# lim0606/pytorch-ardae-vae

Measured on AMD Instinct MI355X. Metric: AR-DAE-VAE train-steps/sec (batch 512, nz_cdae 256) on dbMNIST, higher is better.
Workload: dtype f32; 1 GPU; BASELINE config #2: MNISTIPVAE mlp z=32 h=256 + cDAE mlp-grad h=256 L=3, global batch 512, nz_cdae 256 (131072 rows), dynamic binarisation on device, 1 cDAE + 1 VAE update per step; global_batch=512, nz_cdae=256, per_gpu_batch=512, parallelism=dp1

## Files before the change

### pytorch-ardae-vae_amd/csrc/wgrad_x9.hip

```cpp
#include <stdlib.h>

#include <type_traits>

#include "profile.h"
#include "wgrad.h"
#include "wgrad_wide_tiles.h"

namespace ardae {
namespace {

typedef __bf16 bf16x8 __attribute__((ext_vector_type(8)));
typedef float f32x8 __attribute__((ext_vector_type(8)));

constexpr int XT = 256;
constexpr int XRC = 16;
constexpr int X_PLANE_BYTES = 2 * XT * 16;
constexpr int X_OP_BYTES = 3 * X_PLANE_BYTES;
constexpr int X_BUF_BYTES = 2 * X_OP_BYTES;

__device__ __forceinline__ void xload1(float& dst, unsigned voff, const float* sbase) {
  asm volatile("s_nop 4\n\tglobal_load_dword %0, %1, %2" : "+v"(dst) : "v"(voff), "s"(sbase) : "memory");
}
__device__ __forceinline__ void xload4(f32x4& dst, unsigned voff, const float* sbase) {
  asm volatile("s_nop 4\n\tglobal_load_dwordx4 %0, %1, %2" : "+v"(dst) : "v"(voff), "s"(sbase) : "memory");
}
template <int N>
__device__ __forceinline__ void xwait() { asm volatile("s_waitcnt vmcnt(%0)" : : "n"(N) : "memory"); }
__device__ __forceinline__ void take_landed(const float& loaded, unsigned& top, float& copy) {
  asm volatile("v_and_b32 %0, 0xffff0000, %2\n\tv_mov_b32 %1, %2" : "=&v"(top), "=&v"(copy) : "v"(loaded));
}
__device__ __forceinline__ void take_landed(const f32x4& loaded, f32x4& copy) {
  asm volatile("v_mov_b32 %0, %4\n\tv_mov_b32 %1, %5\n\tv_mov_b32 %2, %6\n\tv_mov_b32 %3, %7"
               : "=&v"(copy[0]), "=&v"(copy[1]), "=&v"(copy[2]), "=&v"(copy[3])
               : "v"(loaded[0]), "v"(loaded[1]), "v"(loaded[2]), "v"(loaded[3]));
}

struct Cut3 { unsigned h, m, l; };
__device__ __forceinline__ Cut3 cut3(float x) {
  Cut3 c;
  c.h = __float_as_uint(x) & 0xffff0000u;
  const float r1 = x - __uint_as_float(c.h);
  c.m = __float_as_uint(r1) & 0xffff0000u;
  c.l = __float_as_uint(r1 - __uint_as_float(c.m));
  return c;
}
__device__ __forceinline__ unsigned pack_hi(unsigned even, unsigned odd) { return __builtin_amdgcn_perm(odd, even, 0x07060302u); }
typedef unsigned u32x4 __attribute__((ext_vector_type(4)));

template <int N, class F>
__device__ __forceinline__ void static_for(F&& f) {
  if constexpr (N > 0) {
    static_for<N - 1>(f);
    f(std::integral_constant<int, N - 1>{});
  }
}
constexpr int X9_PA[9] = {2, 1, 2, 0, 2, 1, 0, 1, 0}, X9_PB[9] = {2, 2, 1, 2, 0, 1, 1, 0, 0};

struct X9Chunk {
  const float* g; const float* x; const float* rs;
  int ldg, ldx;
  float fb, fr;
};

__global__ __launch_bounds__(256, 1) void wgrad_x9_kernel(const WwBatchDev batch) {
  extern __shared__ __attribute__((aligned(16))) unsigned char lds[];
  const int tid = threadIdx.x, lane = tid & 63;
  const int wave = __builtin_amdgcn_readfirstlane(tid >> 6);
  const int l31 = lane & 31, hh = lane >> 5;
  const int wo = wave >> 1, wi = wave & 1;
  const int ti = (int)blockIdx.x / batch.splits, split = (int)blockIdx.x - ti * batch.splits;
  const WwTile T = batch.t[ti];

  const int cpp = T.M / XRC;
  const int ctot = cpp * T.npairs;
  const int cps = (ctot + batch.splits - 1) / batch.splits;
  const int c_begin = split * cps;
  const int c_end = c_begin + cps < ctot ? c_begin + cps : ctot;

  auto chunk_at = [&](int ch) {
    X9Chunk c;
    const int cc = ch < c_end ? ch : c_end - 1;
    const int pr = cc >= cpp ? 1 : 0;
    const int m0 = (cc - pr * cpp) * XRC;
    c.ldg = pr ? T.ldG[1] : T.ldG[0];
    c.ldx = pr ? T.ldX[1] : T.ldX[0];
    c.g = (pr ? T.G[1] : T.G[0]) + (size_t)m0 * c.ldg + T.o0;
    c.x = (pr ? T.X[1] : T.X[0]) + (size_t)m0 * c.ldx + T.i0;
    const bool vec = T.want_vec && pr == T.bias_pair && ch < c_end;
    c.fb = vec ? 1.f : 0.f;
    c.fr = (vec && T.rowscale) ? 1.f : 0.f;
    c.rs = T.rowscale ? T.rowscale + m0 : c.g;
    return c;
  };
  auto issue_loads = [&](const X9Chunk& c, float (&g)[XRC], float (&x)[XRC], f32x4 (&rs)[4]) {
    const float* pg = c.g;
    const float* px = c.x;
#pragma unroll
    for (int j = 0; j < XRC; ++j) {
      xload1(g[j], (unsigned)tid * 4u, pg); pg += c.ldg;
      if ((j & 3) == 3) xload4(rs[j >> 2], 0u, c.rs + (j & ~3));
    }
#pragma unroll
    for (int j = 0; j < XRC; ++j) { xload1(x[j], (unsigned)tid * 4u, px); px += c.ldx; }
  };
  float bsum = 0.f, rsum = 0.f;
  auto write_group = [&](const u32x4& h, const u32x4& m, const u32x4& l, int op, int kg, unsigned char* buf) {
    unsigned char* p = buf + op * X_OP_BYTES + (kg * XT + tid) * 16;
    *reinterpret_cast<u32x4*>(p) = h;
    *reinterpret_cast<u32x4*>(p + X_PLANE_BYTES) = m;
    *reinterpret_cast<u32x4*>(p + 2 * X_PLANE_BYTES) = l;
  };
  auto stage_group = [&](const float (&v)[XRC], int op, int kg, unsigned char* buf) {
    u32x4 h, m, l;
#pragma unroll
    for (int q = 0; q < 4; ++q) {
      const Cut3 e = cut3(v[8 * kg + 2 * q]), o = cut3(v[8 * kg + 2 * q + 1]);
      h[q] = pack_hi(e.h, o.h); m[q] = pack_hi(e.m, o.m); l[q] = pack_hi(e.l, o.l);
    }
    write_group(h, m, l, op, kg, buf);
  };

  f32x16 acc[4][4];
#pragma unroll
  for (int a = 0; a < 4; ++a)
#pragma unroll
    for (int b = 0; b < 4; ++b)
#pragma unroll
      for (int r = 0; r < 16; ++r) acc[a][b][r] = 0.f;

  if (c_begin < c_end) {
    float gc[XRC], xc[XRC];
    f32x4 rsc[4];
#pragma unroll
    for (int j = 0; j < XRC; ++j) gc[j] = xc[j] = 0.f;
#pragma unroll
    for (int q = 0; q < 4; ++q) rsc[q] = f32x4{0.f, 0.f, 0.f, 0.f};
    {
      const X9Chunk c0 = chunk_at(c_begin);
      issue_loads(c0, gc, xc, rsc);
      asm volatile("s_waitcnt vmcnt(0)" ::: "memory");
#pragma unroll
      for (int j = 0; j < XRC; ++j) asm volatile("" : "+v"(gc[j]), "+v"(xc[j]));
#pragma unroll
      for (int q = 0; q < 4; ++q) asm volatile("" : "+v"(rsc[q]));
      {
        float s0 = 0.f, r0 = 0.f;
#pragma unroll
        for (int j = 0; j < XRC; ++j) { s0 += gc[j]; r0 += gc[j] * rsc[j >> 2][j & 3]; }
        bsum += s0 * c0.fb; rsum += r0 * c0.fr;
      }
      stage_group(gc, 0, 0, lds); stage_group(gc, 0, 1, lds); stage_group(xc, 1, 0, lds); stage_group(xc, 1, 1, lds);
      issue_loads(chunk_at(c_begin + 1), gc, xc, rsc);
      __syncthreads();
    }
    int buf = 0;
    bf16x8 Af[3][4], Bf[3][4];
    auto read_plane = [&](auto pp, const unsigned char* from) {
      constexpr int p = decltype(pp)::value;
      static_for<4>([&](auto aa) {
        constexpr int a = decltype(aa)::value;
        Af[p][a] = *reinterpret_cast<const bf16x8*>(from + p * X_PLANE_BYTES + (hh * XT + wo * 128 + a * 32 + l31) * 16);
      });
      static_for<4>([&](auto bb) {
        constexpr int b = decltype(bb)::value;
        Bf[p][b] = *reinterpret_cast<const bf16x8*>(from + X_OP_BYTES + p * X_PLANE_BYTES + (hh * XT + wi * 128 + b * 32 + l31) * 16);
      });
    };
    using I0 = std::integral_constant<int, 0>;
    using I1 = std::integral_constant<int, 1>;
    using I2 = std::integral_constant<int, 2>;
    read_plane(I2{}, lds);
    read_plane(I1{}, lds);
    X9Chunk c1 = chunk_at(c_begin + 1);
#pragma unroll 1
    for (int ch = c_begin; ch < c_end; ++ch) {
      unsigned char* cur = lds + buf * X_BUF_BYTES;
      unsigned char* oth = lds + (buf ^ 1) * X_BUF_BYTES;
      const X9Chunk c2 = chunk_at(ch + 2);
      const float* pgn = c2.g;
      const float* pxn = c2.x;
      u32x4 sh, sm, sl;
      Cut3 ce{0u, 0u, 0u}, co{0u, 0u, 0u};
      float r1 = 0.f, vv = 0.f, cs = 0.f, cr = 0.f;
      f32x4 rsv = {0.f, 0.f, 0.f, 0.f};
      static_for<144>([&](auto nn) {
        constexpr int n = decltype(nn)::value, s = n >> 4, idx = n & 15, a = idx >> 2, b = idx & 3;
        acc[a][b] = __builtin_amdgcn_mfma_f32_32x32x16_bf16(Af[X9_PA[s]][a], Bf[X9_PB[s]][b], acc[a][b], 0, 0, 0);
        __builtin_amdgcn_sched_barrier(0);
        if constexpr (n == 0) {
          read_plane(I0{}, cur);
          __builtin_amdgcn_sched_barrier(0);
        }
        if constexpr (n < 124) {
          constexpr int grp = n / 31, r = n % 31;
          if constexpr (r < 28) {
            constexpr int pr = r / 7, slot = r % 7, e = 8 * grp + 2 * pr + (slot >= 3 ? 1 : 0), op = e >> 4, j = e & 15;
            float& v = op ? xc[j] : gc[j];
            if constexpr (slot == 0 || slot == 3) {
              xwait<35>();
              Cut3& c = slot == 0 ? ce : co;
              take_landed(v, c.h, vv);
              r1 = vv - __uint_as_float(c.h);
              if constexpr (op == 0) cs += vv;
            } else if constexpr (slot == 1 || slot == 4) {
              Cut3& c = slot == 1 ? ce : co;
              c.m = __float_as_uint(r1) & 0xffff0000u;
              c.l = __float_as_uint(r1 - __uint_as_float(c.m));
              if constexpr (op == 0) {
                if constexpr ((j & 3) == 0) { xwait<31>(); take_landed(rsc[j >> 2], rsv); }
                cr += vv * rsv[j & 3];
              }
            } else if constexpr (slot == 2 || slot == 5) {
              if constexpr (op == 0) {
                xload1(v, (unsigned)tid * 4u, pgn); pgn += c2.ldg;
                if constexpr ((j & 3) == 3) xload4(rsc[j >> 2], 0u, c2.rs + (j & ~3));
              } else {
                xload1(v, (unsigned)tid * 4u, pxn); pxn += c2.ldx;
              }
            } else {
              sh[pr] = pack_hi(ce.h, co.h); sm[pr] = pack_hi(ce.m, co.m); sl[pr] = pack_hi(ce.l, co.l);
            }
          } else {
            constexpr int pl = r - 28;
            unsigned char* p = oth + (grp >> 1) * X_OP_BYTES + ((grp & 1) * XT + tid) * 16 + pl * X_PLANE_BYTES;
            *reinterpret_cast<u32x4*>(p) = pl == 0 ? sh : pl == 1 ? sm : sl;
          }
          __builtin_amdgcn_sched_barrier(0);
        }
        if constexpr (n == 124) {
          __syncthreads();
          __builtin_amdgcn_sched_barrier(0);
        }
        if constexpr (n == 125) {
          read_plane(I2{}, oth);
          __builtin_amdgcn_sched_barrier(0);
        }
        if constexpr (n == 128) {
          read_plane(I1{}, oth);
          __builtin_amdgcn_sched_barrier(0);
        }
      });
      bsum += cs * c1.fb; rsum += cr * c1.fr;
      buf ^= 1;
      c1 = c2;
    }
    asm volatile("s_waitcnt vmcnt(0)" ::: "memory");
  }

  float* __restrict__ part = T.partial + (size_t)split * T.O * T.I;
#pragma unroll
  for (int a = 0; a < 4; ++a) {
#pragma unroll
    for (int b = 0; b < 4; ++b) {
      const int i = T.i0 + wi * 128 + b * 32 + l31;
#pragma unroll
      for (int r = 0; r < 16; ++r) {
        const int o = T.o0 + wo * 128 + a * 32 + (r & 3) + 8 * (r >> 2) + 4 * hh;
        part[(size_t)o * T.I + i] = acc[a][b][r];
      }
    }
  }
  if (T.want_vec && T.i0 == 0) {
    T.partial_vec[((size_t)split * 2 + 0) * T.O + T.o0 + tid] = bsum;
    T.partial_vec[((size_t)split * 2 + 1) * T.O + T.o0 + tid] = rsum;
  }
}

}

bool wgrad_x9_eligible(const WgradProblem& p) {
  static const bool off = debug_knob("ARDAE_WGRAD_X9") && atoi(debug_knob("ARDAE_WGRAD_X9")) == 0;
  if (off || p.O % XT || p.I % XT || p.M % XRC || p.M < 64 * 32) return false;
  for (int k = 0; k < p.npairs; ++k)
    if ((int64_t)p.ldG[k] * XRC * 4 >= (int64_t)1 << 31 || (int64_t)p.ldX[k] * XRC * 4 >= (int64_t)1 << 31) return false;
  return true;
}

int launch_wgrad_x9(const WwBatchDev& b, hipStream_t st) {
  static const bool attr_set = [] {
    return hipFuncSetAttribute(reinterpret_cast<const void*>(wgrad_x9_kernel), hipFuncAttributeMaxDynamicSharedMemorySize, 2 * X_BUF_BYTES) == hipSuccess;
  }();
  ARDAE_CHECK_ARG(attr_set, "wgrad_x9: cannot reserve %d bytes of LDS", 2 * X_BUF_BYTES);
  hipLaunchKernelGGL(wgrad_x9_kernel, dim3(b.ntiles * b.splits), dim3(256), 2 * X_BUF_BYTES, st, b);
  return 0;
}

}
```

### scratch/x9_stamps_patch.py

```python
import sys
p='pytorch-ardae-vae_amd/csrc/wgrad_wide_tiles.h'
s=open(p).read()
s=s.replace('  int ntiles, splits;','  int ntiles, splits;\n  unsigned long long* stamps;')
open(p,'w').write(s)
p='pytorch-ardae-vae_amd/csrc/wgrad_x9.hip'
s=open(p).read()
s=s.replace('''      unsigned char* cur = lds + buf * X_BUF_BYTES;''','''      const bool stamp = batch.stamps && blockIdx.x == 7 && ch == c_begin + 20 && tid == 0;
      unsigned long long T0 = 0, T1 = 0, T2 = 0, T3 = 0, TM[9] = {0};
      if (batch.stamps) T0 = __builtin_readcyclecounter();
      unsigned char* cur = lds + buf * X_BUF_BYTES;''',1)
s=s.replace('''        constexpr int n = decltype(nn)::value, s = n >> 4, idx = n & 15, a = idx >> 2, b = idx & 3;''','''        constexpr int n = decltype(nn)::value, s = n >> 4, idx = n & 15, a = idx >> 2, b = idx & 3;
        if constexpr (n == 1) { if (batch.stamps) T1 = __builtin_readcyclecounter(); }
        if constexpr (idx == 15) { if (batch.stamps) TM[s] = __builtin_readcyclecounter(); }
        if constexpr (n == 143) { if (batch.stamps) T2 = __builtin_readcyclecounter(); }''',1)
s=s.replace('''      bsum += cs * c1.fb; rsum += cr * c1.fr;
      buf ^= 1;''','''      bsum += cs * c1.fb; rsum += cr * c1.fr;
      buf ^= 1;
      if (batch.stamps) T3 = __builtin_readcyclecounter();
      if (stamp) { batch.stamps[0] = T0; batch.stamps[1] = T1; batch.stamps[2] = T2; batch.stamps[3] = T3; batch.stamps[4] = __builtin_readcyclecounter(); batch.stamps[5] = __builtin_amdgcn_s_memrealtime();
                   for (int q = 0; q < 9; ++q) batch.stamps[8 + q] = TM[q]; }
      if (batch.stamps && blockIdx.x == 7 && ch == c_begin + 120 && tid == 0) { batch.stamps[6] = __builtin_readcyclecounter(); batch.stamps[7] = __builtin_amdgcn_s_memrealtime(); }''',1)
s=s.replace('''int launch_wgrad_x9(const WwBatchDev& b, hipStream_t st) {''','''int launch_wgrad_x9(const WwBatchDev& b0, hipStream_t st) {
  static unsigned long long* dstamps = nullptr;
  static int calls = 0;
  WwBatchDev b = b0;
  b.stamps = nullptr;
  if (debug_knob("ARDAE_X9_STAMPS")) {
    if (!dstamps) { (void)hipMalloc(&dstamps, 256); (void)hipMemset(dstamps, 0, 256); }
    b.stamps = dstamps;
    if (++calls == 40) {
      (void)hipDeviceSynchronize();
      unsigned long long h[32];
      (void)hipMemcpy(h, dstamps, 256, hipMemcpyDeviceToHost);
      fprintf(stderr, "x9 stamps (cycles): start->MFMA1 %llu, MFMA1->MFMA143 %llu, ->end of trip %llu, barrier %llu; 100 trips: %llu cycles, %llu ticks of 100 MHz; products:", h[1] - h[0], h[2] - h[1], h[3] - h[2], h[4] - h[3], h[6] - h[4], h[7] - h[5]);
      for (int q = 0; q < 9; ++q) fprintf(stderr, " %llu", h[8 + q] - (q ? h[8 + q - 1] : h[1]));
      fprintf(stderr, "\\n");
    }
  }''',1)
open(p,'w').write(s)
```

Measured before the change: 223.5 train-steps/sec.

## Re-schedule x9 wgrad main loop: split LDS stores, spread fragment reads, hoist per-trip setup

New measurement: 225.5 train-steps/sec, median of 6. About the same (+0.9%).

```diff
diff --git a/pytorch-ardae-vae_amd/csrc/wgrad_x9.hip b/pytorch-ardae-vae_amd/csrc/wgrad_x9.hip
--- a/pytorch-ardae-vae_amd/csrc/wgrad_x9.hip
+++ b/pytorch-ardae-vae_amd/csrc/wgrad_x9.hip
@@ -46,6 +46,7 @@
 }
 __device__ __forceinline__ unsigned pack_hi(unsigned even, unsigned odd) { return __builtin_amdgcn_perm(odd, even, 0x07060302u); }
 typedef unsigned u32x4 __attribute__((ext_vector_type(4)));
+typedef unsigned u32x2 __attribute__((ext_vector_type(2)));
 
 template <int N, class F>
 __device__ __forceinline__ void static_for(F&& f) {
@@ -77,19 +78,26 @@
   const int c_begin = split * cps;
   const int c_end = c_begin + cps < ctot ? c_begin + cps : ctot;
 
+  const float fb_on = T.want_vec ? 1.f : 0.f, fr_on = (T.want_vec && T.rowscale) ? 1.f : 0.f;
+  auto chunk_rows = [&](int ch, int& pr, int& m0) {
+    const int cc = ch < c_end ? ch : c_end - 1;
+    pr = cc >= cpp ? 1 : 0;
+    m0 = (cc - pr * cpp) * XRC;
+  };
+  auto chunk_ld = [&](int ch, X9Chunk& c, int pr) {
+    c.ldg = pr ? T.ldG[1] : T.ldG[0];
+    c.ldx = pr ? T.ldX[1] : T.ldX[0];
+    const bool vec = (pr == T.bias_pair) & (ch < c_end);
+    c.fb = vec ? fb_on : 0.f;
+    c.fr = vec ? fr_on : 0.f;
+  };
+  auto chunk_g = [&](X9Chunk& c, int pr, int m0) { c.g = (pr ? T.G[1] : T.G[0]) + (size_t)m0 * c.ldg + T.o0; };
+  auto chunk_x = [&](X9Chunk& c, int pr, int m0) { c.x = (pr ? T.X[1] : T.X[0]) + (size_t)m0 * c.ldx + T.i0; };
+  auto chunk_rs = [&](X9Chunk& c, int m0) { c.rs = T.rowscale ? T.rowscale + m0 : c.g; };
   auto chunk_at = [&](int ch) {
     X9Chunk c;
-    const int cc = ch < c_end ? ch : c_end - 1;
-    const int pr = cc >= cpp ? 1 : 0;
-    const int m0 = (cc - pr * cpp) * XRC;
-    c.ldg = pr ? T.ldG[1] : T.ldG[0];
-    c.ldx = pr ? T.ldX[1] : T.ldX[0];
-    c.g = (pr ? T.G[1] : T.G[0]) + (size_t)m0 * c.ldg + T.o0;
-    c.x = (pr ? T.X[1] : T.X[0]) + (size_t)m0 * c.ldx + T.i0;
-    const bool vec = T.want_vec && pr == T.bias_pair && ch < c_end;
-    c.fb = vec ? 1.f : 0.f;
-    c.fr = (vec && T.rowscale) ? 1.f : 0.f;
-    c.rs = T.rowscale ? T.rowscale + m0 : c.g;
+    int pr, m0;
+    chunk_rows(ch, pr, m0); chunk_ld(ch, c, pr); chunk_g(c, pr, m0); chunk_x(c, pr, m0); chunk_rs(c, m0);
     return c;
   };
   auto issue_loads = [&](const X9Chunk& c, float (&g)[XRC], float (&x)[XRC], f32x4 (&rs)[4]) {
@@ -153,46 +161,48 @@
       issue_loads(chunk_at(c_begin + 1), gc, xc, rsc);
       __syncthreads();
     }
-    int buf = 0;
     bf16x8 Af[3][4], Bf[3][4];
-    auto read_plane = [&](auto pp, const unsigned char* from) {
-      constexpr int p = decltype(pp)::value;
-      static_for<4>([&](auto aa) {
-        constexpr int a = decltype(aa)::value;
-        Af[p][a] = *reinterpret_cast<const bf16x8*>(from + p * X_PLANE_BYTES + (hh * XT + wo * 128 + a * 32 + l31) * 16);
-      });
-      static_for<4>([&](auto bb) {
-        constexpr int b = decltype(bb)::value;
-        Bf[p][b] = *reinterpret_cast<const bf16x8*>(from + X_OP_BYTES + p * X_PLANE_BYTES + (hh * XT + wi * 128 + b * 32 + l31) * 16);
-      });
+    auto read_frag = [&](auto pp, auto kk, const unsigned char* from) {
+      constexpr int p = decltype(pp)::value, k = decltype(kk)::value;
+      if constexpr (k < 4) Af[p][k] = *reinterpret_cast<const bf16x8*>(from + p * X_PLANE_BYTES + (hh * XT + wo * 128 + k * 32 + l31) * 16);
+      else Bf[p][k - 4] = *reinterpret_cast<const bf16x8*>(from + X_OP_BYTES + p * X_PLANE_BYTES + (hh * XT + wi * 128 + (k - 4) * 32 + l31) * 16);
     };
     using I0 = std::integral_constant<int, 0>;
     using I1 = std::integral_constant<int, 1>;
     using I2 = std::integral_constant<int, 2>;
-    read_plane(I2{}, lds);
-    read_plane(I1{}, lds);
-    X9Chunk c1 = chunk_at(c_begin + 1);
+    static_for<8>([&](auto kk) { read_frag(I2{}, kk, lds); });
+    static_for<8>([&](auto kk) { read_frag(I1{}, kk, lds); });
+    X9Chunk c2 = chunk_at(c_begin + 2);
+    const float* pgn = c2.g;
+    const float* pxn = c2.x;
+    float fb1, fr1;
+    { const X9Chunk c1 = chunk_at(c_begin + 1); fb1 = c1.fb; fr1 = c1.fr; }
+    unsigned char* cur = lds;
+    unsigned char* oth = lds + X_BUF_BYTES;
+    u32x4 sh, sm, sl;
+    Cut3 ce{0u, 0u, 0u}, co{0u, 0u, 0u};
+    float r1 = 0.f, vv = 0.f, cs = 0.f, cr = 0.f;
+    f32x4 rsv = {0.f, 0.f, 0.f, 0.f};
+    int npr = 0, nm0 = 0;
+    auto store_half = [&](auto gg, auto pl_, auto half_) {
+      constexpr int grp = decltype(gg)::value, pl = decltype(pl_)::value, half = decltype(half_)::value;
+      unsigned char* p = oth + (grp >> 1) * X_OP_BYTES + ((grp & 1) * XT + tid) * 16 + pl * X_PLANE_BYTES + half * 8;
+      const u32x4& v = pl == 0 ? sh : pl == 1 ? sm : sl;
+      *reinterpret_cast<u32x2*>(p) = u32x2{v[2 * half], v[2 * half + 1]};
+    };
 #pragma unroll 1
     for (int ch = c_begin; ch < c_end; ++ch) {
-      unsigned char* cur = lds + buf * X_BUF_BYTES;
-      unsigned char* oth = lds + (buf ^ 1) * X_BUF_BYTES;
-      const X9Chunk c2 = chunk_at(ch + 2);
-      const float* pgn = c2.g;
-      const float* pxn = c2.x;
-      u32x4 sh, sm, sl;
-      Cut3 ce{0u, 0u, 0u}, co{0u, 0u, 0u};
-      float r1 = 0.f, vv = 0.f, cs = 0.f, cr = 0.f;
-      f32x4 rsv = {0.f, 0.f, 0.f, 0.f};
       static_for<144>([&](auto nn) {
         constexpr int n = decltype(nn)::value, s = n >> 4, idx = n & 15, a = idx >> 2, b = idx & 3;
         acc[a][b] = __builtin_amdgcn_mfma_f32_32x32x16_bf16(Af[X9_PA[s]][a], Bf[X9_PB[s]][b], acc[a][b], 0, 0, 0);
         __builtin_amdgcn_sched_barrier(0);
-        if constexpr (n == 0) {
-          read_plane(I0{}, cur);
-          __builtin_amdgcn_sched_barrier(0);
-        }
-        if constexpr (n < 124) {
-          constexpr int grp = n / 31, r = n % 31;
+        if constexpr (n == 0 || n == 3 || n == 4 || n == 6) {
+          constexpr int k0 = n == 0 ? 0 : n == 3 ? 2 : n == 4 ? 4 : 6;
+          read_frag(I0{}, std::integral_constant<int, k0>{}, cur);
+          read_frag(I0{}, std::integral_constant<int, k0 + 1>{}, cur);
+        }
+        if constexpr (n < 120) {
+          constexpr int grp = n / 30, r = n % 30;
           if constexpr (r < 28) {
             constexpr int pr = r / 7, slot = r % 7, e = 8 * grp + 2 * pr + (slot >= 3 ? 1 : 0), op = e >> 4, j = e & 15;
             float& v = op ? xc[j] : gc[j];
@@ -201,14 +211,17 @@
               Cut3& c = slot == 0 ? ce : co;
               take_landed(v, c.h, vv);
               r1 = vv - __uint_as_float(c.h);
-              if constexpr (op == 0) cs += vv;
+              if constexpr (op == 0) { cs += vv; asm volatile("" : "+v"(cs)); }
             } else if constexpr (slot == 1 || slot == 4) {
               Cut3& c = slot == 1 ? ce : co;
               c.m = __float_as_uint(r1) & 0xffff0000u;
               c.l = __float_as_uint(r1 - __uint_as_float(c.m));
               if constexpr (op == 0) {
                 if constexpr ((j & 3) == 0) { xwait<31>(); take_landed(rsc[j >> 2], rsv); }
-                cr += vv * rsv[j & 3];
+                float sg = vv * rsv[j & 3];
+                asm volatile("" : "+v"(sg));
+                cr += sg;
+                asm volatile("" : "+v"(cr));
               }
             } else if constexpr (slot == 2 || slot == 5) {
               if constexpr (op == 0) {
@@ -219,30 +232,40 @@
               }
             } else {
               sh[pr] = pack_hi(ce.h, co.h); sm[pr] = pack_hi(ce.m, co.m); sl[pr] = pack_hi(ce.l, co.l);
+              if constexpr (pr == 0 && grp > 0) store_half(std::integral_constant<int, (grp > 0 ? grp - 1 : 0)>{}, I2{}, I1{});
+              if constexpr (pr > 0) store_half(std::integral_constant<int, grp>{}, std::integral_constant<int, (pr > 0 ? pr - 1 : 0)>{}, I0{});
             }
           } else {
-            constexpr int pl = r - 28;
-            unsigned char* p = oth + (grp >> 1) * X_OP_BYTES + ((grp & 1) * XT + tid) * 16 + pl * X_PLANE_BYTES;
-            *reinterpret_cast<u32x4*>(p) = pl == 0 ? sh : pl == 1 ? sm : sl;
+            store_half(std::integral_constant<int, grp>{}, std::integral_constant<int, r - 28>{}, I1{});
           }
-          __builtin_amdgcn_sched_barrier(0);
-        }
-        if constexpr (n == 124) {
-          __syncthreads();
-          __builtin_amdgcn_sched_barrier(0);
-        }
-        if constexpr (n == 125) {
-          read_plane(I2{}, oth);
-          __builtin_amdgcn_sched_barrier(0);
-        }
-        if constexpr (n == 128) {
-          read_plane(I1{}, oth);
-          __builtin_amdgcn_sched_barrier(0);
-        }
+        }
+        if constexpr (n == 120) store_half(std::integral_constant<int, 3>{}, I2{}, I1{});
+        if constexpr (n == 122) {
+          bsum += cs * fb1; rsum += cr * fr1;
+          cs = 0.f; cr = 0.f;
+        }
+        if constexpr (n == 124) asm volatile("s_waitcnt lgkmcnt(0)\n\ts_barrier" ::: "memory");
+        if constexpr (n >= 125 && n < 133) {
+          constexpr int q = 2 * (n - 125);
+          static_for<2>([&](auto tt) {
+            constexpr int k = q + decltype(tt)::value;
+            if constexpr (k == 0) read_frag(I2{}, I0{}, oth);
+            else if constexpr (k < 5) read_frag(I2{}, std::integral_constant<int, (k < 5 ? k + 3 : 0)>{}, oth);
+            else if constexpr (k < 8) read_frag(I2{}, std::integral_constant<int, (k < 8 ? k - 4 : 0)>{}, oth);
+            else read_frag(I1{}, std::integral_constant<int, (k >= 8 ? k - 8 : 0)>{}, oth);
+          });
+        }
+        if constexpr (n == 133) {
+          chunk_rows(ch + 3, npr, nm0);
+          asm volatile("" : "+s"(nm0));
+        }
+        if constexpr (n == 134) { fb1 = c2.fb; fr1 = c2.fr; chunk_ld(ch + 3, c2, npr); asm volatile("" : "+s"(c2.ldg), "+s"(c2.ldx), "+v"(c2.fb), "+v"(c2.fr)); }
+        if constexpr (n == 135) { chunk_g(c2, npr, nm0); pgn = c2.g; asm volatile("" : "+s"(pgn)); }
+        if constexpr (n == 136) { chunk_x(c2, npr, nm0); pxn = c2.x; asm volatile("" : "+s"(pxn)); }
+        if constexpr (n == 137) { chunk_rs(c2, nm0); asm volatile("" : "+s"(c2.rs)); }
+        if constexpr (n == 138) { unsigned char* t = cur; cur = oth; oth = t; }
+        if constexpr (n < 143) __builtin_amdgcn_sched_barrier(0);
       });
-      bsum += cs * c1.fb; rsum += cr * c1.fr;
-      buf ^= 1;
-      c1 = c2;
     }
     asm volatile("s_waitcnt vmcnt(0)" ::: "memory");
   }
diff --git a/scratch/x9_stamps_patch.py b/scratch/x9_stamps_patch.py
--- a/scratch/x9_stamps_patch.py
+++ b/scratch/x9_stamps_patch.py
@@ -1,40 +1,47 @@
 import sys
-p='pytorch-ardae-vae_amd/csrc/wgrad_wide_tiles.h'
-s=open(p).read()
-s=s.replace('  int ntiles, splits;','  int ntiles, splits;\n  unsigned long long* stamps;')
-open(p,'w').write(s)
-p='pytorch-ardae-vae_amd/csrc/wgrad_x9.hip'
-s=open(p).read()
-s=s.replace('''      unsigned char* cur = lds + buf * X_BUF_BYTES;''','''      const bool stamp = batch.stamps && blockIdx.x == 7 && ch == c_begin + 20 && tid == 0;
-      unsigned long long T0 = 0, T1 = 0, T2 = 0, T3 = 0, TM[9] = {0};
-      if (batch.stamps) T0 = __builtin_readcyclecounter();
-      unsigned char* cur = lds + buf * X_BUF_BYTES;''',1)
-s=s.replace('''        constexpr int n = decltype(nn)::value, s = n >> 4, idx = n & 15, a = idx >> 2, b = idx & 3;''','''        constexpr int n = decltype(nn)::value, s = n >> 4, idx = n & 15, a = idx >> 2, b = idx & 3;
-        if constexpr (n == 1) { if (batch.stamps) T1 = __builtin_readcyclecounter(); }
-        if constexpr (idx == 15) { if (batch.stamps) TM[s] = __builtin_readcyclecounter(); }
-        if constexpr (n == 143) { if (batch.stamps) T2 = __builtin_readcyclecounter(); }''',1)
-s=s.replace('''      bsum += cs * c1.fb; rsum += cr * c1.fr;
-      buf ^= 1;''','''      bsum += cs * c1.fb; rsum += cr * c1.fr;
-      buf ^= 1;
-      if (batch.stamps) T3 = __builtin_readcyclecounter();
-      if (stamp) { batch.stamps[0] = T0; batch.stamps[1] = T1; batch.stamps[2] = T2; batch.stamps[3] = T3; batch.stamps[4] = __builtin_readcyclecounter(); batch.stamps[5] = __builtin_amdgcn_s_memrealtime();
-                   for (int q = 0; q < 9; ++q) batch.stamps[8 + q] = TM[q]; }
-      if (batch.stamps && blockIdx.x == 7 && ch == c_begin + 120 && tid == 0) { batch.stamps[6] = __builtin_readcyclecounter(); batch.stamps[7] = __builtin_amdgcn_s_memrealtime(); }''',1)
-s=s.replace('''int launch_wgrad_x9(const WwBatchDev& b, hipStream_t st) {''','''int launch_wgrad_x9(const WwBatchDev& b0, hipStream_t st) {
-  static unsigned long long* dstamps = nullptr;
-  static int calls = 0;
-  WwBatchDev b = b0;
-  b.stamps = nullptr;
-  if (debug_knob("ARDAE_X9_STAMPS")) {
-    if (!dstamps) { (void)hipMalloc(&dstamps, 256); (void)hipMemset(dstamps, 0, 256); }
-    b.stamps = dstamps;
-    if (++calls == 40) {
-      (void)hipDeviceSynchronize();
-      unsigned long long h[32];
-      (void)hipMemcpy(h, dstamps, 256, hipMemcpyDeviceToHost);
-      fprintf(stderr, "x9 stamps (cycles): start->MFMA1 %llu, MFMA1->MFMA143 %llu, ->end of trip %llu, barrier %llu; 100 trips: %llu cycles, %llu ticks of 100 MHz; products:", h[1] - h[0], h[2] - h[1], h[3] - h[2], h[4] - h[3], h[6] - h[4], h[7] - h[5]);
-      for (int q = 0; q < 9; ++q) fprintf(stderr, " %llu", h[8 + q] - (q ? h[8 + q - 1] : h[1]));
-      fprintf(stderr, "\\n");
-    }
-  }''',1)
-open(p,'w').write(s)
+
+root = sys.argv[1] if len(sys.argv) > 1 else "."
+at = [int(v) for v in (sys.argv[2] if len(sys.argv) > 2 else "0,1,16,32,48,64,80,96,112,124,125,128,133,143").split(",")]
+assert at[0] == 0 and at == sorted(at) and at[-1] < 144 and len(at) <= 20
+p = root + "/pytorch-ardae-vae_amd/csrc/wgrad_x9.hip"
+s = open(p).read()
+
+
+def sub(old, new):
+    global s
+    assert s.count(old) == 1, old
+    s = s.replace(old, new)
+
+
+sub("__global__ __launch_bounds__(256, 1) void wgrad_x9_kernel(",
+    "constexpr int X9_NS = %d;\nconstexpr int X9_AT[X9_NS] = {%s};\n" % (len(at), ", ".join(map(str, at)))
+    + "constexpr int x9_slot(int n) { for (int k = 0; k < X9_NS; ++k) if (X9_AT[k] == n) return k; return -1; }\n"
+    + "__device__ unsigned x9_stamp_out[32];\n"
+    + "__global__ __launch_bounds__(256, 1) void wgrad_x9_kernel(")
+sub("#pragma unroll 1\n    for (int ch = c_begin; ch < c_end; ++ch) {\n",
+    "    unsigned TS[X9_NS] = {0}, TS21 = 0, TS120 = 0;\n#pragma unroll 1\n    for (int ch = c_begin; ch < c_end; ++ch) {\n")
+sub("        constexpr int n = decltype(nn)::value, s = n >> 4, idx = n & 15, a = idx >> 2, b = idx & 3;\n",
+    "        constexpr int n = decltype(nn)::value, s = n >> 4, idx = n & 15, a = idx >> 2, b = idx & 3;\n"
+    "        if constexpr (x9_slot(n) >= 0) {\n"
+    "          const unsigned t = (unsigned)__builtin_readcyclecounter();\n"
+    "          TS[x9_slot(n) >= 0 ? x9_slot(n) : 0] = ch == c_begin + 20 ? t : TS[x9_slot(n) >= 0 ? x9_slot(n) : 0];\n"
+    "          if constexpr (n == 0) { TS21 = ch == c_begin + 21 ? t : TS21; TS120 = ch == c_begin + 120 ? t : TS120; }\n"
+    "        }\n")
+sub('    asm volatile("s_waitcnt vmcnt(0)" ::: "memory");      // (the re-loads of the last trip: nothing uses them)\n',
+    '    asm volatile("s_waitcnt vmcnt(0)" ::: "memory");      // (the re-loads of the last trip: nothing uses them)\n'
+    "    if (blockIdx.x == 7 && tid == 0) {\n"
+    "      static_for<X9_NS>([&](auto kk) { x9_stamp_out[decltype(kk)::value] = TS[decltype(kk)::value]; });\n"
+    "      x9_stamp_out[30] = TS21; x9_stamp_out[31] = TS120;\n"
+    "    }\n")
+sub("  hipLaunchKernelGGL(wgrad_x9_kernel, dim3(b.ntiles * b.splits), dim3(256), 2 * X_BUF_BYTES, st, b);\n",
+    "  hipLaunchKernelGGL(wgrad_x9_kernel, dim3(b.ntiles * b.splits), dim3(256), 2 * X_BUF_BYTES, st, b);\n"
+    "  static int calls = 0;\n"
+    '  if (debug_knob("ARDAE_X9_STAMPS") && ++calls == 40) {\n'
+    "    (void)hipDeviceSynchronize();\n"
+    "    unsigned h[32];\n"
+    "    (void)hipMemcpyFromSymbol(h, HIP_SYMBOL(x9_stamp_out), sizeof h);\n"
+    '    fprintf(stderr, "x9 stamps, cycles (trip 20 of workgroup 7): whole trip %u; 100 trips %u = %.1f per trip; from the stamp in front of MFMA n to the next:", h[30] - h[0], h[31] - h[0], (h[31] - h[0]) / 100.0);\n'
+    '    for (int k = 0; k < X9_NS; ++k) fprintf(stderr, " [%d] %u", X9_AT[k], (k + 1 < X9_NS ? h[k + 1] : h[30]) - h[k]);\n'
+    '    fprintf(stderr, "\\n");\n'
+    "  }\n")
+open(p, "w").write(s)
```
